# Zilong-Li/BaseVarC

Measured on AMD Instinct MI355X. Metric: sites/sec at N=1e6 samples; achieved HBM GB/s vs roofline, higher is better.
Workload: dtype f64

## Files before the change

basevarc_amd/csrc/bvc_context.hip:

```cpp
#include <cmath>
#include <cstdlib>
#include <cstring>
#include <mutex>
#include <new>

#include "bvc_ctx.h"

hipError_t sync_streams(bvc_ctx *ctx)
{
    hipError_t first = hipSuccess;
    for (hipStream_t s : streams_of(ctx)) {
        const hipError_t e = hipStreamSynchronize(s);
        if (first == hipSuccess) first = e;
    }
    for (bool &p : ctx->em_pending) p = false;
    return first;
}

int drain_on_error(bvc_ctx *ctx, int code)
{
    (void)sync_streams(ctx);
    (void)hipGetLastError();
    return code;
}
// ... 81 lines not shown
        if (c >= r.first && c + n <= r.first + r.second) return true;
    return false;
}

namespace {
struct Knob {
    const char *key, *env;
    int lo, hi, step, dflt;
    int LaunchState::*member;
    bool takes(int v) const { return v >= lo && v <= hi && (v - lo) % step == 0; }
};
const Knob kKnobs[] = {
    {"em_waves_per_cu", "BVC_EM_WAVES_PER_CU", 0, 32, 1, 0, &LaunchState::em_waves_per_cu},
    {"em_wpb", "BVC_EM_WPB", 1, 4, 3, 4, &LaunchState::em_wpb},
    {"hist_split", "BVC_HIST_SPLIT", 0, 64, 1, 0, &LaunchState::hist_split},
    {"group_pipe", "BVC_GROUP_PIPE", 0, 1, 1, 1, &LaunchState::group_pipe},
    {"group_copies_log2", "BVC_GROUP_LOG2C", -1, 5, 1, -1, &LaunchState::group_log2c},
    {"group_big_lds", "BVC_GROUP_BIG_LDS", 0, 1, 1, 1, &LaunchState::group_big_lds},
    {"group_h16", "BVC_GROUP_H16", 0, 1, 1, 0, &LaunchState::group_h16},
    {"em_streams", "BVC_EM_STREAMS", 0, 3, 1, 0, &LaunchState::em_streams},
    {"em_engine", "BVC_EM_ENGINE", 0, 1, 1, 0, &LaunchState::em_engine},
    {"em_tiny_regions", "BVC_EM_TINY_REGIONS", 0, 1, 1, 0, &LaunchState::em_tiny_regions},
    {"em_prune", "BVC_EM_PRUNE", 0, 1, 1, 1, &LaunchState::em_prune},
    {"host_chunk_kib", nullptr, 1, 1 << 21, 1, 1 << 19, &LaunchState::host_chunk_kib},
};
}

extern "C" {

const char *bvc_version(void) { return "libbvc 0.3.0 (gfx950)"; }
// ... 252 lines not shown
```

basevarc_amd/csrc/bvc_internal.h:

```cpp
#pragma once
#include <hip/hip_runtime.h>
#include <stdint.h>

#include <vector>

#include "../../include/bvc.h"

namespace bvc {

struct LaunchState {
    int n_cu = 256;
    int em_waves_per_cu = 0;
    int em_wpb = 4;
    int hist_split = 0;
    int host_chunk_kib = 1 << 19;
    int em_streams = 0;
    int group_pipe = 1;
    int group_log2c = -1;
    int group_big_lds = 1;
    int group_h16 = 0;
    int em_engine = 0;
    int em_tiny_regions = 0;
    int em_prune = 1;
    int dbg_levels = 0;
    mutable uint32_t em_epoch = 0;
    struct RaisedLds { const void *kernel; size_t bytes; };
    mutable std::vector<RaisedLds> lds_raised;
};

// ... 8 lines not shown
        at += round256(count * sizeof(T) + pad);
        return p;
    }
};

hipError_t raise_lds(const LaunchState &st, const void *kernel, size_t bytes);

struct QualLut {
    double a[128];
    double e[128];
    double e_empty;
    double log_e[128];
    double log_a[128];
};

hipError_t launch_hist_dense(LaunchState &st, hipStream_t stream, int64_t n_sites, int64_t n_samples, int64_t row_stride,
                             const int8_t *bases, const int8_t *quals, const uint8_t *group_of_sample,
                             int n_groups, uint32_t *counts, int split, int64_t *group_scratch = nullptr,
                             uint8_t *hist_of_sample = nullptr);
constexpr int kGroupScratchWords = BVC_MAX_GROUPS + 4;
inline size_t group_redo_offset(int64_t n_samples) { return ((size_t)n_samples + 255) & ~(size_t)255; }
inline size_t group_labels_bytes(int64_t n_samples, int64_t n_sites) { return group_redo_offset(n_samples) + (size_t)n_sites + 256; }
int choose_hist_split(const LaunchState &st, int64_t n_sites, int64_t n_samples);

hipError_t launch_hist_packed(LaunchState &st, hipStream_t stream, int64_t n_sites, int64_t n_samples, int64_t row_stride,
                              const uint8_t *packed, uint32_t *counts, int split);
hipError_t launch_hist_packed_groups(LaunchState &st, hipStream_t stream, int64_t n_sites, int64_t n_samples,
                                     int64_t row_stride, const uint8_t *packed, const uint8_t *group_of_sample, int n_groups,
                                     uint32_t *counts, int64_t *group_scratch, uint8_t *hist_of_sample);
hipError_t launch_pack_dense(hipStream_t stream, int64_t n_sites, int64_t n_samples, int64_t stride_in, const int8_t *bases,
                             const int8_t *quals, int64_t stride_out, uint8_t *packed, unsigned long long *bad);

hipError_t launch_stream_read(hipStream_t stream, const void *src, int64_t bytes, uint32_t *sink);

hipError_t launch_hist_csr(LaunchState &st, hipStream_t stream, int64_t n_sites, const int64_t *offsets,
                           const int8_t *bases, const int8_t *quals, uint32_t *counts);

inline bool uses_item_engine(const LaunchState &st, double min_af) { return st.em_engine != 1 && min_af > 0.0; }
hipError_t launch_lrt(const LaunchState &st, hipStream_t stream, int64_t n_sites, const uint32_t *counts,
                      int64_t hist_stride, const int8_t *ref_base, double min_af, const QualLut *lut,
                      const int8_t *comb, const uint8_t *n_comb, bvc_site_result *results, bool shared = false,
// ... 75 lines not shown
```

basevarc_amd/csrc/bvc_lrt.hip:

```cpp
#include "bvc_ctx.h"

namespace {

int em_stream_count(const bvc_ctx *ctx, int by_default) { return ctx->ls.em_streams > 0 ? ctx->ls.em_streams : by_default; }

hipStream_t em_stream(bvc_ctx *ctx, int by_default)
{
    const int n = em_stream_count(ctx, by_default);
    const int k = (int)(ctx->side_flip++ % (unsigned)n);
    return k == 0 ? ctx->side : (k == 1 ? ctx->side_b : ctx->side_c);
}

int ensure_joined(bvc_ctx *ctx, DevBuf &buf, size_t need)
{
    if (need > buf.cap) {
        const int rc = join_side(ctx);
        if (rc != BVC_OK) return rc;
    }
    return ensure(ctx, buf, need);
}

int em_scratch_for(bvc_ctx *ctx, int slot, int64_t n_sites, double min_af, void **out, int n_groups = 0)
{
    *out = nullptr;
    if (!uses_item_engine(ctx->ls, min_af)) return BVC_OK;
    const size_t need = n_groups > 0 ? em_group_scratch_bytes(n_sites, n_groups) : em_items_scratch_bytes(n_sites);
    DevBuf &buf = n_groups > 0 ? ctx->d_emg[slot] : ctx->d_em[slot];
    const int rc = ensure_joined(ctx, buf, need);
    if (rc != BVC_OK) return rc;
    *out = buf.p;
    return BVC_OK;
}

template <class Stage1, class Stage2>
int run_stages(bvc_ctx *ctx, int64_t n_sites, int n_groups, bool zero_counts, double min_af, int em_streams, Stage1 stage1,
               Stage2 stage2)
{
    const size_t cbytes = (size_t)n_sites * BVC_NCLASS * sizeof(uint32_t), gbytes = cbytes * (size_t)(n_groups + 1);
    const int buf = ctx->overlap ? ctx->flip : 0;
    if (ctx->overlap) ctx->flip = (ctx->flip + 1) % bvc_ctx::kRing;
    DevBuf &cnt = ctx->d_cnt[buf], &grp = ctx->d_grp[buf];
    int rc = ensure_joined(ctx, cnt, cbytes);
    if (rc == BVC_OK && n_groups > 0) rc = ensure_joined(ctx, grp, gbytes);
    RingSlot slot;
    if (rc == BVC_OK) rc = em_scratch_for(ctx, buf, n_sites, min_af, &slot.em);
    if (rc == BVC_OK && n_groups > 0) rc = em_scratch_for(ctx, buf, n_sites, min_af, &slot.emg, n_groups);
    if (rc != BVC_OK) return rc;
    slot.counts = reinterpret_cast<uint32_t *>(cnt.p);
    if (n_groups > 0) slot.grp = reinterpret_cast<uint32_t *>(grp.p);
    bvc_ctx::Triple t{nullptr, nullptr, nullptr, nullptr, n_sites};
    const bool timed = ctx->profiling && take_timing_events(ctx, t);
    auto enqueue = [&]() -> int {
        if (ctx->overlap && ctx->em_pending[buf]) {
            BVC_HIP(ctx, hipStreamWaitEvent(ctx->stream, ctx->ev_em_done[buf], 0));
            ctx->em_pending[buf] = false;
        }
        if (zero_counts) BVC_HIP(ctx, hipMemsetAsync(slot.counts, 0, cbytes, ctx->stream));
        if (timed) BVC_HIP(ctx, hipEventRecord(t.a, ctx->stream));
        BVC_HIP(ctx, stage1(n_groups > 0 ? slot.grp : slot.counts));
        if (timed) BVC_HIP(ctx, hipEventRecord(t.b, ctx->stream));
        hipStream_t s2 = ctx->stream;
        if (ctx->overlap) {
            s2 = em_stream(ctx, em_streams);
            BVC_HIP(ctx, hipEventRecord(ctx->ev_hist_done[buf], ctx->stream));
            BVC_HIP(ctx, hipStreamWaitEvent(s2, ctx->ev_hist_done[buf], 0));
        }
        if (timed) BVC_HIP(ctx, hipEventRecord(t.c, s2));
        const int rc2 = stage2(s2, slot);
        if (rc2 != BVC_OK) return rc2;
        if (timed) {
            BVC_HIP(ctx, hipEventRecord(t.d, s2));
            ctx->ev_pending.push_back(t);
            t = bvc_ctx::Triple{nullptr, nullptr, nullptr, nullptr, 0};
            if (ctx->ev_pending.size() > 256) reap_timing(ctx, false);
        }
        if (ctx->overlap) {
            BVC_HIP(ctx, hipEventRecord(ctx->ev_em_done[buf], s2));
            ctx->em_pending[buf] = true;
        }
        return BVC_OK;
    };
    rc = enqueue();
    give_back(ctx, t);
    return rc;
}

template <class Stage1>
int run_two_stages(bvc_ctx *ctx, int64_t n_sites, bool zero_counts, bool long_rows, Stage1 stage1,
                   const int8_t *ref_base, double min_af, const int8_t *comb, const uint8_t *n_comb,
                   bvc_site_result *results, int em_streams_long_rows = 1)
{
    return run_stages(ctx, n_sites, 0, zero_counts, min_af, long_rows ? em_streams_long_rows : 2, stage1,
                      [&](hipStream_t s2, const RingSlot &slot) -> int {
                          const bool shared = ctx->overlap && long_rows;
                          BVC_HIP(ctx, launch_lrt(ctx->ls, s2, n_sites, slot.counts, BVC_NCLASS, ref_base, min_af, ctx->d_lut, comb,
                                                  n_comb, results, shared, 0, slot.em));
                          return BVC_OK;
                      });
}

int run_dense_device(bvc_ctx *ctx, int64_t n_sites, int64_t n_samples, int64_t row_stride,
                     const int8_t *bases, const int8_t *quals, const int8_t *ref_base, double min_af,
                     bvc_site_result *results)
{
    const int split = choose_hist_split(ctx->ls, n_sites, n_samples);
    return run_two_stages(ctx, n_sites, split > 1, n_samples >= 200000,
                          [&](uint32_t *counts) {
                              return launch_hist_dense(ctx->ls, ctx->stream, n_sites, n_samples, row_stride, bases, quals,
                                                       nullptr, 0, counts, split);
                          },
                          ref_base, min_af, nullptr, nullptr, results);
}

int run_packed_device(bvc_ctx *ctx, int64_t n_sites, int64_t n_samples, int64_t row_stride, const uint8_t *packed,
                      const int8_t *ref_base, double min_af, bvc_site_result *results)
{
    const int split = choose_hist_split(ctx->ls, n_sites, n_samples);
    return run_two_stages(ctx, n_sites, split > 1, n_samples >= 200000,
                          [&](uint32_t *counts) {
                              return launch_hist_packed(ctx->ls, ctx->stream, n_sites, n_samples, row_stride, packed, counts, split);
                          },
                          ref_base, min_af, nullptr, nullptr, results, 2);
}

template <class Upload, class Compute>
int run_chunks(bvc_ctx *ctx, int64_t n_sites, int64_t chunk, Upload upload, Compute compute)
{
    int set = 0;
    int rc = upload(set, (int64_t)0, n_sites < chunk ? n_sites : chunk);
    if (rc != BVC_OK) return drain_on_error(ctx, rc);
    BVC_HIP_D(ctx, hipEventRecord(ctx->ev_upload[set], ctx->copy));
    for (int64_t s0 = 0; s0 < n_sites; s0 += chunk, set ^= 1) {
        const int64_t ns = n_sites - s0 < chunk ? n_sites - s0 : chunk;
// ... 61 lines not shown
                int rc = device(ns, d);
                return rc == BVC_OK ? join_side(ctx) : rc;
            }
            BVC_HIP(ctx, hipMemcpyAsync(results + s0, d.res, (size_t)ns * sizeof(bvc_site_result), hipMemcpyDeviceToHost, ctx->stream));
            if (n_groups > 0)
                BVC_HIP(ctx, hipMemcpyAsync(grp_results + s0 * n_groups, d.gres, (size_t)ns * n_groups * sizeof(bvc_group_result),
                                            hipMemcpyDeviceToHost, ctx->stream));
            return BVC_OK;
        });
}

template <class Stage1>
int run_group_stages(bvc_ctx *ctx, int64_t ns, int n_groups, bool long_rows, Stage1 stage1, const int8_t *r, double min_af,
                     bvc_site_result *res, bvc_group_result *gres)
{
    return run_stages(ctx, ns, n_groups, false, min_af, 2, stage1, [&](hipStream_t s2, const RingSlot &slot) -> int {
        BVC_HIP(ctx, launch_sum_groups(s2, ns, n_groups + 1, slot.grp, slot.counts));
        const bool shared = ctx->overlap && long_rows;
        const int per_launch = kGroupSharedWavesPerCu / em_stream_count(ctx, 2) > 2 ? kGroupSharedWavesPerCu / em_stream_count(ctx, 2) : 2;
        BVC_HIP(ctx, launch_lrt(ctx->ls, s2, ns, slot.counts, BVC_NCLASS, r, min_af, ctx->d_lut, nullptr, nullptr, res, shared, per_launch,
                                slot.em));
        BVC_HIP(ctx, launch_lrt_groups(ctx->ls, s2, ns, n_groups, slot.grp, r, min_af, ctx->d_lut, res, gres, shared, per_launch, slot.emg));
        return BVC_OK;
    });
}

int run_csr_groups_device(bvc_ctx *ctx, int64_t n_sites, const int64_t *offsets, const int8_t *bases, const int8_t *quals,
                          const int32_t *sample_of_obs, const int8_t *ref_base, double min_af, const uint8_t *group_of_sample,
                          int64_t n_samples, int32_t n_groups, bvc_site_result *results, bvc_group_result *grp_results)
{
    return run_group_stages(ctx, n_sites, n_groups, false,
// ... 25 lines not shown
    if (rc != BVC_OK) return rc;
    BVC_HIP_D(ctx, hipMemcpyAsync(d_o, offsets, (size_t)(n_sites + 1) * 8, hipMemcpyHostToDevice, ctx->stream));
    BVC_HIP_D(ctx, hipMemcpyAsync(d_r, ref_base, (size_t)n_sites, hipMemcpyHostToDevice, ctx->stream));
    if (n_samples) BVC_HIP_D(ctx, hipMemcpyAsync(d_g, group_of_sample, (size_t)n_samples, hipMemcpyHostToDevice, ctx->stream));
    for (int a = 0; a < n_arrays && total; ++a)
        BVC_HIP_D(ctx, hipMemcpyAsync(arrays[a].dev, arrays[a].host, total * arrays[a].elem, hipMemcpyHostToDevice, ctx->stream));
    rc = device(d_o, d_r, d_g, d_res, d_gres);
    if (rc == BVC_OK) rc = join_side(ctx);
    if (rc != BVC_OK) return drain_on_error(ctx, rc);
    BVC_HIP_D(ctx, hipMemcpyAsync(results, d_res, (size_t)n_sites * sizeof(bvc_site_result), hipMemcpyDeviceToHost, ctx->stream));
    BVC_HIP_D(ctx, hipMemcpyAsync(grp_results, d_gres, (size_t)n_sites * n_groups * sizeof(bvc_group_result), hipMemcpyDeviceToHost, ctx->stream));
    BVC_HIP_D(ctx, hipStreamSynchronize(ctx->stream));
    return BVC_OK;
}

}

int run_csr_device(bvc_ctx *ctx, int64_t n_sites, const int64_t *offsets, const int8_t *bases, const int8_t *quals,
                   const int8_t *ref_base, double min_af, const int8_t *comb, const uint8_t *n_comb,
                   bvc_site_result *results)
{
    return run_two_stages(ctx, n_sites, false, false,
                          [&](uint32_t *counts) { return launch_hist_csr(ctx->ls, ctx->stream, n_sites, offsets, bases, quals, counts); },
                          ref_base, min_af, comb, n_comb, results);
}

int run_csr_labels_device(bvc_ctx *ctx, int64_t n_sites, const int64_t *offsets, const uint8_t *obs, const uint8_t *quals,
                          const uint8_t *group_of_obs, const int8_t *ref_base, double min_af, int32_t n_groups,
                          bvc_site_result *results, bvc_group_result *grp_results)
{
    return run_group_stages(ctx, n_sites, n_groups, false,
                            [&](uint32_t *gp) {
                                return launch_hist_csr_labels(ctx->ls, ctx->stream, n_sites, offsets, obs, quals, group_of_obs, n_groups, gp);
                            },
                            ref_base, min_af, results, grp_results);
}

// ... 49 lines not shown
    BVC_HIP(ctx, launch_pack_dense(ctx->stream, n_sites, n_samples, row_stride, bases, quals, packed_stride, packed, d_bad));
    unsigned long long bad = 0;
    BVC_HIP(ctx, hipMemcpyAsync(&bad, d_bad, sizeof bad, hipMemcpyDeviceToHost, ctx->stream));
    BVC_HIP(ctx, hipStreamSynchronize(ctx->stream));
    *n_unrepresentable = (int64_t)bad;
    return BVC_OK;
}

int bvc_hist_dense_packed(bvc_ctx *ctx, int64_t n_sites, int64_t n_samples, int64_t row_stride, const uint8_t *packed,
                          uint32_t *counts, uint32_t flags)
{
    int rc = check_dense(ctx, n_sites, n_samples, row_stride, n_samples ? (const void *)packed : (const void *)counts, counts, counts, counts);
    if (rc != BVC_OK) return rc;
    if (!(flags & BVC_PTR_DEVICE)) return fail(ctx, BVC_ERR_ARG, "bvc_hist_dense_packed takes device pointers");
    if (n_sites == 0) return BVC_OK;
    const int split = choose_hist_split(ctx->ls, n_sites, n_samples);
    if (split > 1) BVC_HIP(ctx, hipMemsetAsync(counts, 0, (size_t)n_sites * BVC_NCLASS * sizeof(uint32_t), ctx->stream));
    BVC_HIP(ctx, launch_hist_packed(ctx->ls, ctx->stream, n_sites, n_samples, row_stride, packed, counts, split));
    return BVC_OK;
}

int bvc_hist_dense(bvc_ctx *ctx, int64_t n_sites, int64_t n_samples, int64_t row_stride,
                   const int8_t *bases, const int8_t *quals, uint32_t *counts, uint32_t flags)
{
    int rc = check_dense(ctx, n_sites, n_samples, row_stride, n_samples ? (const void *)bases : (const void *)counts,
                         n_samples ? (const void *)quals : (const void *)counts, counts, counts);
    if (rc != BVC_OK) return rc;
    if (n_sites == 0) return BVC_OK;
    const int split = choose_hist_split(ctx->ls, n_sites, n_samples);
    const size_t cbytes = (size_t)n_sites * BVC_NCLASS * sizeof(uint32_t);
    if (flags & BVC_PTR_DEVICE) {
        if (split > 1) BVC_HIP(ctx, hipMemsetAsync(counts, 0, cbytes, ctx->stream));
        BVC_HIP(ctx, launch_hist_dense(ctx->ls, ctx->stream, n_sites, n_samples, row_stride, bases, quals, nullptr, 0, counts, split));
        return BVC_OK;
    }
    const size_t bytes = n_samples ? (size_t)(n_sites - 1) * (size_t)row_stride + (size_t)n_samples : 0;
    int8_t *d_b, *d_q;
    uint32_t *d_c;
    rc = carve(ctx, ctx->d_stage[0], 256, [&](Layout &L) {
        d_b = L.take<int8_t>(bytes);
        d_q = L.take<int8_t>(bytes);
        d_c = L.take<uint32_t>((size_t)n_sites * BVC_NCLASS);
    });
    if (rc != BVC_OK) return rc;
    if (bytes) BVC_HIP(ctx, hipMemcpyAsync(d_b, bases, bytes, hipMemcpyHostToDevice, ctx->stream));
    if (bytes) BVC_HIP(ctx, hipMemcpyAsync(d_q, quals, bytes, hipMemcpyHostToDevice, ctx->stream));
    if (split > 1) BVC_HIP(ctx, hipMemsetAsync(d_c, 0, cbytes, ctx->stream));
    BVC_HIP(ctx, launch_hist_dense(ctx->ls, ctx->stream, n_sites, n_samples, row_stride, d_b, d_q, nullptr, 0, d_c, split));
    BVC_HIP(ctx, hipMemcpyAsync(counts, d_c, cbytes, hipMemcpyDeviceToHost, ctx->stream));
    BVC_HIP(ctx, hipStreamSynchronize(ctx->stream));
    return BVC_OK;
}

static int check_comb_host(bvc_ctx *ctx, int64_t n_sites, const int8_t *base_comb, const uint8_t *n_comb)
{
    for (int64_t s = 0; s < n_sites; ++s) {
        if (n_comb[s] > 4) return fail(ctx, BVC_ERR_ARG, "n_comb > 4");
        for (int c = 0; c < n_comb[s]; ++c)
            if (base_comb[s * 4 + c] < 0 || base_comb[s * 4 + c] > 3) return fail(ctx, BVC_ERR_ARG, "base_comb entry outside 0..3");
    }
    return BVC_OK;
}
// ... 246 lines not shown
    if (n_groups < 1 || n_groups > BVC_MAX_GROUPS) return fail(ctx, BVC_ERR_ARG, "n_groups must be 1..32");
    if (!group_of_sample || !grp_results) return fail(ctx, BVC_ERR_ARG, "null group pointer");
    if (n_sites == 0) return BVC_OK;
    auto run_device = [&](int64_t ns, const int8_t *b, const int8_t *q, const int8_t *r, const uint8_t *g,
                          bvc_site_result *res, bvc_group_result *gres) -> int {
        const size_t lbytes = group_labels_bytes(n_samples, ns);
        int rc2 = ensure_joined(ctx, ctx->d_grp_labels, lbytes);
        if (rc2 != BVC_OK) return rc2;
        uint8_t *labels = reinterpret_cast<uint8_t *>(ctx->d_grp_labels.p);
        return run_group_stages(ctx, ns, n_groups, n_samples >= 200000,
                                [&](uint32_t *gp) {
                                    if (packed)
                                        return launch_hist_packed_groups(ctx->ls, ctx->stream, ns, n_samples, row_stride,
                                                                         reinterpret_cast<const uint8_t *>(b), g, n_groups, gp,
                                                                         ctx->d_grp_scratch, labels);
                                    return launch_hist_dense(ctx->ls, ctx->stream, ns, n_samples, row_stride, b, q, g, n_groups, gp, 1,
                                                             ctx->d_grp_scratch, labels);
                                },
                                r, min_af, res, gres);
    };

    if (flags & BVC_PTR_DEVICE)
        return run_device(n_sites, bases, quals, ref_base, group_of_sample, results, grp_results);

    const int8_t *rows[2] = {bases, quals};
    return run_dense_host(ctx, n_sites, n_samples, row_stride, packed ? 1 : 2, rows, ref_base, group_of_sample, n_groups, results,
                          grp_results, [&](int64_t ns, const DenseSet &d) {
                              return run_device(ns, d.rows[0], d.rows[1], d.ref, d.labels, d.res, d.gres);
                          });
}

// ... 20 lines not shown
```

basevarc_amd/csrc/hist_kernel.hip:

```cpp
#include "bvc_device.h"
#include "bvc_internal.h"

#include <utility>

namespace bvc {
namespace {

#ifndef BVC_HIST_THREADS
#define BVC_HIST_THREADS 512
#endif
#ifndef BVC_HIST_UNROLL
#define BVC_HIST_UNROLL 2
#endif
constexpr int kHistThreads = BVC_HIST_THREADS;
constexpr int kCopies = 32;
constexpr int kLdsWords = BVC_NCLASS * kCopies;
constexpr int kUnroll = BVC_HIST_UNROLL;
constexpr int kGroupDepth = 2;
constexpr int64_t kWaveRowMax = 16384;

typedef uint32_t u32x4 __attribute__((ext_vector_type(4)));

template <int BYTE>
__device__ __forceinline__ uint32_t shl_byte(uint32_t word, uint32_t shift)
// ... 193 lines not shown
        const int64_t c = cb + tid + (int64_t)u * kHistThreads;
        b[u] = u32x4{0xFFFFFFFFu, 0xFFFFFFFFu, 0xFFFFFFFFu, 0xFFFFFFFFu};
        q[u] = u32x4{0u, 0u, 0u, 0u};
        if (c < c1) {
            b[u] = __builtin_nontemporal_load(&bv[c]);
            q[u] = __builtin_nontemporal_load(&qv[c]);
        }
    }
#pragma unroll
    for (int u = 0; u < kUnroll; ++u) {
        const int64_t wave_first = cb + (tid & ~63) + (int64_t)u * kHistThreads;
        if (wave_first < c1) count_chunk(hist, b[u], q[u], lane_off);
    }
}

template <bool ALIGNED>
__global__ __launch_bounds__(kHistThreads) void hist_dense_kernel(
    int64_t n_sites, int64_t n_samples, int64_t row_stride, const int8_t *__restrict__ bases,
    const int8_t *__restrict__ quals, uint32_t *__restrict__ counts, int split)
{
    BVC_POISON_LDS();
    extern __shared__ __attribute__((aligned(16))) uint32_t hist[];
    const int tid = threadIdx.x;
    const uint32_t lane_off = (uint32_t)(tid & (kCopies - 1));
    __builtin_amdgcn_s_setprio(3);

    clear_lds(hist, kLdsWords, tid);
    __syncthreads();

    const int64_t n_work = n_sites * split;
    for (int64_t w = blockIdx.x; w < n_work; w += gridDim.x) {
        const int64_t site = w / split;
        const int part = (int)(w % split);
        const int8_t *brow = bases + site * row_stride;
        const int8_t *qrow = quals + site * row_stride;
        const int64_t n16 = n_samples >> 4;
        constexpr int64_t kBlockChunks = (int64_t)kUnroll * kHistThreads;

        if (ALIGNED) {
            const u32x4 *bv = reinterpret_cast<const u32x4 *>(brow);
            const u32x4 *qv = reinterpret_cast<const u32x4 *>(qrow);
            for (int64_t cb = (int64_t)part * kBlockChunks; cb < n16; cb += (int64_t)split * kBlockChunks) {
                if (cb + kBlockChunks <= n16) {
                    u32x4 b[kUnroll], q[kUnroll];
                    load_block(bv, qv, cb + tid, b, q);
#pragma unroll
                    for (int u = 0; u < kUnroll; ++u) count_chunk(hist, b[u], q[u], lane_off);
                } else {
// ... 4 lines not shown
            for (int64_t cb = (int64_t)part * kBlockChunks; cb < n16; cb += (int64_t)split * kBlockChunks) {
                const int64_t i1 = (cb + kBlockChunks < n16 ? cb + kBlockChunks : n16) * 16;
                count_bytes(hist, brow, qrow, cb * 16, i1, tid, lane_off);
            }
        }
        if (part == split - 1) count_bytes(hist, brow, qrow, n16 << 4, n_samples, tid, lane_off);
        __syncthreads();

        for (int key = tid; key < BVC_NCLASS; key += kHistThreads) {
            const uint32_t s = fold_class<kCopies>(hist, key);
            if (split == 1) counts[site * BVC_NCLASS + key] = s;
            else if (s) atomicAdd(&counts[site * BVC_NCLASS + key], s);
        }
        __syncthreads();
    }
}


__global__ __launch_bounds__(kHistThreads) void hist_dense_groups_bytes_kernel(
    int64_t n_sites, int64_t n_samples, int64_t row_stride, const int8_t *__restrict__ bases,
    const int8_t *__restrict__ quals, const uint8_t *__restrict__ group_of_sample, int n_groups, int log2c,
    uint32_t *__restrict__ grp_counts, const int64_t *__restrict__ bounds)
{
    BVC_POISON_LDS();
    extern __shared__ __attribute__((aligned(16))) uint32_t hist[];
    if (bounds && bounds[0] == 0) return;
    const int tid = threadIdx.x;
    const int n_hist = n_groups + 1;
    const int words = (n_hist * BVC_NCLASS) << log2c;
    const uint32_t lane_off = (uint32_t)tid & ((1u << log2c) - 1u);
// ... 457 lines not shown
{
    for (int64_t i = i0 + tid; i < i1; i += kHistThreads) lds_add_one(((uint32_t)row[i] << 8) + lane_base);
}

__device__ __forceinline__ uint32_t fold_packed_class(uint32_t *hist, int key)
{
    const int q = key & 127;
    if (q >= 64) return 0;
    const uint32_t sum = fold_class<kPackedCopies>(hist, ((key >> 7) << 6) | q);
    return q == 63 ? 0u : sum;
}

template <bool ALIGNED>
__global__ __launch_bounds__(kHistThreads) void hist_packed_kernel(
    int64_t n_sites, int64_t n_samples, int64_t row_stride, const uint8_t *__restrict__ packed,
    uint32_t *__restrict__ counts, int split)
{
    BVC_POISON_LDS();
    extern __shared__ __attribute__((aligned(16))) uint32_t hist[];
    const int tid = threadIdx.x;
    const uint32_t lane_base = lds_address(hist) + ((uint32_t)(tid & (kPackedCopies - 1)) << 2);
    const bool at_zero = (lds_address(hist) & 0xFFFFu) == 0u;
    __builtin_amdgcn_s_setprio(3);
    clear_lds(hist, kPackedLdsWords, tid);
    __syncthreads();

    uint32_t a0 = lane_base, a1 = lane_base, a2 = lane_base, a3 = lane_base;
    const int64_t n_work = n_sites * split;
    for (int64_t w = blockIdx.x; w < n_work; w += gridDim.x) {
        const int64_t site = w / split;
        const int part = (int)(w % split);
        const uint8_t *row = packed + site * row_stride;
        const int64_t n16 = (ALIGNED && at_zero) ? n_samples >> 4 : 0;
        constexpr int64_t kBlockChunks = (int64_t)kPackedUnroll * kHistThreads;
        if (ALIGNED && at_zero) {
            const u32x4 *rv = reinterpret_cast<const u32x4 *>(row);
            for (int64_t cb = (int64_t)part * kBlockChunks; cb < n16; cb += (int64_t)split * kBlockChunks) {
                u32x4 v[kPackedUnroll];
                if (cb + kBlockChunks <= n16) {
                    load_block(rv, cb + tid, v);
                } else {
                    load_partial_block(rv, cb + tid, n16, v);
                }
#pragma unroll
                for (int u = 0; u < kPackedUnroll; ++u) {
                    count_packed_chunk(a0, a1, a2, a3, v[u]);
                }
            }
        }
        if (part == split - 1)
            for (int64_t i = (n16 << 4) + tid; i < n_samples; i += kHistThreads)
                lds_add_one(((uint32_t)row[i] << 8) + lane_base);
        __syncthreads();
        for (int key = tid; key < BVC_NCLASS; key += kHistThreads) {
            const uint32_t sum = fold_packed_class(hist, key);
            if (split == 1) counts[site * BVC_NCLASS + key] = sum;
            else if (sum) atomicAdd(&counts[site * BVC_NCLASS + key], sum);
        }
        __syncthreads();
    }
}

template <bool ALIGNED>
__global__ __launch_bounds__(kHistThreads) void hist_packed_ranges_kernel(
    int64_t n_sites, int64_t row_stride, const uint8_t *__restrict__ packed, int n_hist,
    const int64_t *__restrict__ scratch, uint32_t *__restrict__ grp_counts)
{
    BVC_POISON_LDS();
    extern __shared__ __attribute__((aligned(16))) uint32_t hist[];
    if (scratch[0] != 0) return;
    uint8_t *real_h = reinterpret_cast<uint8_t *>(&hist[kPackedLdsWords]);
    int &n_real_s = *reinterpret_cast<int *>(&hist[kPackedLdsWords + 16]);
    const int tid = threadIdx.x;
    const uint32_t lane_base = lds_address(hist) + ((uint32_t)(tid & (kPackedCopies - 1)) << 2);
    const bool at_zero = (lds_address(hist) & 0xFFFFu) == 0u;
// ... 367 lines not shown
    for (; i + 3 * stride < n16; i += 4 * stride) {
        const u32x4 a = __builtin_nontemporal_load(&src[i]), b = __builtin_nontemporal_load(&src[i + stride]);
        const u32x4 c = __builtin_nontemporal_load(&src[i + 2 * stride]), d = __builtin_nontemporal_load(&src[i + 3 * stride]);
        acc ^= a.x ^ a.y ^ a.z ^ a.w ^ b.x ^ b.y ^ b.z ^ b.w ^ c.x ^ c.y ^ c.z ^ c.w ^ d.x ^ d.y ^ d.z ^ d.w;
    }
    for (; i < n16; i += stride) { const u32x4 a = __builtin_nontemporal_load(&src[i]); acc ^= a.x ^ a.y ^ a.z ^ a.w; }
    if (acc == 0x9E3779B9u) sink[0] = acc;
}

}

#ifdef BVC_CHECK_LDS
BVC_DEFINE_DEBUG_READER(debug_read_hist)
#endif

hipError_t launch_stream_read(hipStream_t stream, const void *src, int64_t bytes, uint32_t *sink)
{
    const int64_t n16 = bytes / 16;
    if (n16 <= 0) return hipSuccess;
    int64_t blocks = (n16 + 4 * 512 - 1) / (4 * 512);
    if (blocks > 16384) blocks = 16384;
    hipLaunchKernelGGL(stream_read_kernel, dim3((unsigned)blocks), dim3(512), 0, stream, reinterpret_cast<const u32x4 *>(src), n16, sink);
    return hipGetLastError();
}

int choose_hist_split(const LaunchState &st, int64_t n_sites, int64_t n_samples)
{
    if (st.hist_split > 0) return st.hist_split;
    const int64_t want = (int64_t)st.n_cu * 4;
    if (n_sites >= want || n_samples < (1 << 16)) return 1;
    int64_t split = (want + n_sites - 1) / n_sites;
    const int64_t max_split = n_samples / (1 << 15);
    if (split > max_split) split = max_split;
    if (split < 1) split = 1;
    if (split > 64) split = 64;
    return (int)split;
}

hipError_t raise_lds(const LaunchState &st, const void *kernel, size_t bytes)
{
    for (LaunchState::RaisedLds &done : st.lds_raised)
        if (done.kernel == kernel) {
            if (done.bytes >= bytes) return hipSuccess;
            const hipError_t e = hipFuncSetAttribute(kernel, hipFuncAttributeMaxDynamicSharedMemorySize, (int)bytes);
            if (e == hipSuccess) done.bytes = bytes;
            return e;
        }
    const hipError_t e = hipFuncSetAttribute(kernel, hipFuncAttributeMaxDynamicSharedMemorySize, (int)bytes);
    if (e == hipSuccess) st.lds_raised.push_back({kernel, bytes});
    return e;
}

constexpr size_t kLdsBytes = (size_t)kLdsWords * sizeof(uint32_t);
static_assert(kPackedLdsWords == kLdsWords, "kLdsBytes serves the packed kernels too");
constexpr size_t kBigLdsBytes = 144 * 1024;
constexpr size_t kGroupLdsMax = (size_t)(BVC_MAX_GROUPS + 1) * BVC_NCLASS * sizeof(uint32_t);

static unsigned grid_cap(int64_t n, int64_t cap = 4096) { return (unsigned)(n < cap ? n : cap); }

template <class... P, class... A>
static hipError_t launch(const LaunchState &st, hipStream_t stream, void (*kernel)(P...), unsigned grid, int block, size_t lds,
                         size_t attr_bytes, A... args)
{
    if (attr_bytes) {
        const hipError_t e = raise_lds(st, reinterpret_cast<const void *>(kernel), attr_bytes);
        if (e != hipSuccess) return e;
    }
    hipLaunchKernelGGL(kernel, dim3(grid), dim3(block), lds, stream, static_cast<P>(args)...);
    return hipGetLastError();
}

using Log2cs = std::make_integer_sequence<int, 6>;
template <bool PIPE, int... L>
// ... 31 lines not shown
                                int n_groups, int64_t *group_scratch, uint8_t *hist_of_sample, int slots, size_t big_tail,
                                Ranges launch_ranges, GroupPlan *plan)
{
    if (!group_scratch || !hist_of_sample) return hipErrorInvalidValue;
    hipError_t e = hipMemsetAsync(group_scratch, 0, (size_t)kGroupScratchWords * sizeof(int64_t), stream);
    if (e != hipSuccess) return e;
    e = launch(st, stream, group_bounds_kernel, grid_cap((n_samples + 255) / 256, 1024), 256, 0, 0, group_of_sample, n_samples,
               n_groups, group_scratch, hist_of_sample);
    if (e != hipSuccess) return e;
    *plan = plan_group_copies(st, n_groups + 1, slots, big_tail);
    return launch_ranges();
}

hipError_t launch_hist_dense(LaunchState &st, hipStream_t stream, int64_t n_sites, int64_t n_samples, int64_t row_stride,
                             const int8_t *bases, const int8_t *quals, const uint8_t *group_of_sample,
                             int n_groups, uint32_t *counts, int split, int64_t *group_scratch, uint8_t *hist_of_sample)
{
    if (n_sites <= 0) return hipSuccess;
    const bool aligned = ((reinterpret_cast<uintptr_t>(bases) | reinterpret_cast<uintptr_t>(quals)) & 15u) == 0 &&
                         (row_stride & 15) == 0;
    if (group_of_sample) {
        const int n_hist = n_groups + 1;
        if (n_samples <= 0)
            return hipMemsetAsync(counts, 0, (size_t)n_sites * n_hist * BVC_NCLASS * sizeof(uint32_t), stream);
        GroupPlan g;
        hipError_t e = group_prelude(st, stream, group_of_sample, n_samples, n_groups, group_scratch, hist_of_sample, BVC_NCLASS, 16, [&] {
            return launch(st, stream, aligned ? hist_dense_ranges_kernel<true> : hist_dense_ranges_kernel<false>,
                          grid_cap(n_sites * n_hist), kHistThreads, kLdsBytes, kLdsBytes, n_sites, n_samples, row_stride, bases, quals,
                          n_hist, group_scratch, counts);
        }, &g);
        if (e != hipSuccess) return e;
// ... 1 lines not shown
            return launch(st, stream, hist_dense_groups_bytes_kernel, grid_cap(n_sites), kHistThreads, g.lds, kGroupLdsMax, n_sites,
                          n_samples, row_stride, bases, quals, group_of_sample, n_groups, g.log2c, counts, group_scratch);
        const uint8_t *only = nullptr;
        if (g.big >= 0 && g.log2c < 3) {
            uint8_t *redo = hist_of_sample + group_redo_offset(n_samples);
            e = launch(st, stream, g.big == 4 ? hist_dense_groups_slots_kernel<4> : (g.big == 3 ? hist_dense_groups_slots_kernel<3> : hist_dense_groups_slots_kernel<2>),
                       grid_cap(n_sites), 1024, g.big_lds, kBigLdsBytes, n_sites, n_samples, row_stride, bases, quals, hist_of_sample,
                       n_groups, counts, group_scratch, redo);
            if (e != hipSuccess) return e;
            only = redo;
        }
        return launch(st, stream, st.group_pipe ? dense_groups_instance<true>(g.log2c, Log2cs{}) : dense_groups_instance<false>(g.log2c, Log2cs{}),
                      grid_cap(n_sites), kHistThreads, g.lds, kGroupLdsMax, n_sites, n_samples, row_stride, bases, quals, hist_of_sample,
                      n_groups, counts, group_scratch, only);
    }
    if (split == 1 && n_samples <= kWaveRowMax && n_sites >= (int64_t)st.n_cu * 2 * kCsrWaves)
        return launch(st, stream, aligned ? hist_wave_kernel<true, true> : hist_wave_kernel<false, true>,
                      grid_cap((n_sites + kCsrWaves - 1) / kCsrWaves, 8192), kHistThreads, 0, 0, n_sites, nullptr, n_samples, row_stride,
                      bases, quals, counts);
    return launch(st, stream, aligned ? hist_dense_kernel<true> : hist_dense_kernel<false>, grid_cap(n_sites * split), kHistThreads,
                  kLdsBytes, kLdsBytes, n_sites, n_samples, row_stride, bases, quals, counts, split);
}

hipError_t launch_hist_packed(LaunchState &st, hipStream_t stream, int64_t n_sites, int64_t n_samples, int64_t row_stride,
                              const uint8_t *packed, uint32_t *counts, int split)
{
    if (n_sites <= 0) return hipSuccess;
    const bool aligned = (reinterpret_cast<uintptr_t>(packed) & 15u) == 0 && (row_stride & 15) == 0;
    return launch(st, stream, aligned ? hist_packed_kernel<true> : hist_packed_kernel<false>, grid_cap(n_sites * split), kHistThreads,
                  kLdsBytes, kLdsBytes, n_sites, n_samples, row_stride, packed, counts, split);
}

hipError_t launch_hist_packed_groups(LaunchState &st, hipStream_t stream, int64_t n_sites, int64_t n_samples,
                                     int64_t row_stride, const uint8_t *packed, const uint8_t *group_of_sample, int n_groups,
                                     uint32_t *counts, int64_t *group_scratch, uint8_t *hist_of_sample)
{
    if (n_sites <= 0) return hipSuccess;
    const int n_hist = n_groups + 1;
    if (n_samples <= 0)
        return hipMemsetAsync(counts, 0, (size_t)n_sites * n_hist * BVC_NCLASS * sizeof(uint32_t), stream);
    const bool aligned = (reinterpret_cast<uintptr_t>(packed) & 15u) == 0 && (row_stride & 15) == 0;
    GroupPlan g;
    hipError_t e = group_prelude(st, stream, group_of_sample, n_samples, n_groups, group_scratch, hist_of_sample, kPackedSlots, 0, [&] {
        return launch(st, stream, aligned ? hist_packed_ranges_kernel<true> : hist_packed_ranges_kernel<false>, grid_cap(n_sites * n_hist),
                      kHistThreads, kLdsBytes + 256, kLdsBytes + 256, n_sites, row_stride, packed, n_hist, group_scratch, counts);
// ... 44 lines not shown
```

Before: 3.340 million.

## Split only tail sites across blocks in histogram kernels to balance last wave

Replaces the uniform per-site split factor with a HistSplit that processes most sites whole and splits only the remainder sites (n_sites mod 2*n_cu) into several parts. This targets the tail-wave imbalance where the last partial wave of blocks leaves CUs idle. Only the split rows are zeroed before the kernel, rather than the whole counts buffer. In exchange, tail sites need atomic accumulation into global counts and some launches get larger grids. A compile-time clock probe is also added.

```diff
diff --git a/basevarc_amd/csrc/bvc_context.hip b/basevarc_amd/csrc/bvc_context.hip
--- a/basevarc_amd/csrc/bvc_context.hip
+++ b/basevarc_amd/csrc/bvc_context.hip
@@ -119,6 +119,7 @@
     {"em_waves_per_cu", "BVC_EM_WAVES_PER_CU", 0, 32, 1, 0, &LaunchState::em_waves_per_cu},
     {"em_wpb", "BVC_EM_WPB", 1, 4, 3, 4, &LaunchState::em_wpb},
     {"hist_split", "BVC_HIST_SPLIT", 0, 64, 1, 0, &LaunchState::hist_split},
+    {"hist_tail_split", "BVC_HIST_TAIL_SPLIT", 0, 64, 1, 0, &LaunchState::hist_tail_split},
     {"group_pipe", "BVC_GROUP_PIPE", 0, 1, 1, 1, &LaunchState::group_pipe},
     {"group_copies_log2", "BVC_GROUP_LOG2C", -1, 5, 1, -1, &LaunchState::group_log2c},
     {"group_big_lds", "BVC_GROUP_BIG_LDS", 0, 1, 1, 1, &LaunchState::group_big_lds},
diff --git a/basevarc_amd/csrc/bvc_internal.h b/basevarc_amd/csrc/bvc_internal.h
--- a/basevarc_amd/csrc/bvc_internal.h
+++ b/basevarc_amd/csrc/bvc_internal.h
@@ -13,6 +13,7 @@
     int em_waves_per_cu = 0;
     int em_wpb = 4;
     int hist_split = 0;
+    int hist_tail_split = 0;
     int host_chunk_kib = 1 << 19;
     int em_streams = 0;
     int group_pipe = 1;
@@ -51,17 +52,18 @@
     double log_a[128];
 };
 
+struct HistSplit { int64_t n_whole; int parts; };
 hipError_t launch_hist_dense(LaunchState &st, hipStream_t stream, int64_t n_sites, int64_t n_samples, int64_t row_stride,
                              const int8_t *bases, const int8_t *quals, const uint8_t *group_of_sample,
-                             int n_groups, uint32_t *counts, int split, int64_t *group_scratch = nullptr,
+                             int n_groups, uint32_t *counts, HistSplit hs, int64_t *group_scratch = nullptr,
                              uint8_t *hist_of_sample = nullptr);
 constexpr int kGroupScratchWords = BVC_MAX_GROUPS + 4;
 inline size_t group_redo_offset(int64_t n_samples) { return ((size_t)n_samples + 255) & ~(size_t)255; }
 inline size_t group_labels_bytes(int64_t n_samples, int64_t n_sites) { return group_redo_offset(n_samples) + (size_t)n_sites + 256; }
-int choose_hist_split(const LaunchState &st, int64_t n_sites, int64_t n_samples);
+HistSplit choose_hist_split(const LaunchState &st, int64_t n_sites, int64_t n_samples);
 
 hipError_t launch_hist_packed(LaunchState &st, hipStream_t stream, int64_t n_sites, int64_t n_samples, int64_t row_stride,
-                              const uint8_t *packed, uint32_t *counts, int split);
+                              const uint8_t *packed, uint32_t *counts, HistSplit hs);
 hipError_t launch_hist_packed_groups(LaunchState &st, hipStream_t stream, int64_t n_sites, int64_t n_samples,
                                      int64_t row_stride, const uint8_t *packed, const uint8_t *group_of_sample, int n_groups,
                                      uint32_t *counts, int64_t *group_scratch, uint8_t *hist_of_sample);
diff --git a/basevarc_amd/csrc/bvc_lrt.hip b/basevarc_amd/csrc/bvc_lrt.hip
--- a/basevarc_amd/csrc/bvc_lrt.hip
+++ b/basevarc_amd/csrc/bvc_lrt.hip
@@ -33,7 +33,7 @@
 }
 
 template <class Stage1, class Stage2>
-int run_stages(bvc_ctx *ctx, int64_t n_sites, int n_groups, bool zero_counts, double min_af, int em_streams, Stage1 stage1,
+int run_stages(bvc_ctx *ctx, int64_t n_sites, int n_groups, int64_t zero_from, double min_af, int em_streams, Stage1 stage1,
                Stage2 stage2)
 {
     const size_t cbytes = (size_t)n_sites * BVC_NCLASS * sizeof(uint32_t), gbytes = cbytes * (size_t)(n_groups + 1);
@@ -55,7 +55,9 @@
             BVC_HIP(ctx, hipStreamWaitEvent(ctx->stream, ctx->ev_em_done[buf], 0));
             ctx->em_pending[buf] = false;
         }
-        if (zero_counts) BVC_HIP(ctx, hipMemsetAsync(slot.counts, 0, cbytes, ctx->stream));
+        if (zero_from < n_sites)
+            BVC_HIP(ctx, hipMemsetAsync(slot.counts + zero_from * BVC_NCLASS, 0, (size_t)(n_sites - zero_from) * BVC_NCLASS * sizeof(uint32_t),
+                                        ctx->stream));
         if (timed) BVC_HIP(ctx, hipEventRecord(t.a, ctx->stream));
         BVC_HIP(ctx, stage1(n_groups > 0 ? slot.grp : slot.counts));
         if (timed) BVC_HIP(ctx, hipEventRecord(t.b, ctx->stream));
@@ -86,11 +88,11 @@
 }
 
 template <class Stage1>
-int run_two_stages(bvc_ctx *ctx, int64_t n_sites, bool zero_counts, bool long_rows, Stage1 stage1,
+int run_two_stages(bvc_ctx *ctx, int64_t n_sites, int64_t zero_from, bool long_rows, Stage1 stage1,
                    const int8_t *ref_base, double min_af, const int8_t *comb, const uint8_t *n_comb,
                    bvc_site_result *results, int em_streams_long_rows = 1)
 {
-    return run_stages(ctx, n_sites, 0, zero_counts, min_af, long_rows ? em_streams_long_rows : 2, stage1,
+    return run_stages(ctx, n_sites, 0, zero_from, min_af, long_rows ? em_streams_long_rows : 2, stage1,
                       [&](hipStream_t s2, const RingSlot &slot) -> int {
                           const bool shared = ctx->overlap && long_rows;
                           BVC_HIP(ctx, launch_lrt(ctx->ls, s2, n_sites, slot.counts, BVC_NCLASS, ref_base, min_af, ctx->d_lut, comb,
@@ -103,8 +105,8 @@
                      const int8_t *bases, const int8_t *quals, const int8_t *ref_base, double min_af,
                      bvc_site_result *results)
 {
-    const int split = choose_hist_split(ctx->ls, n_sites, n_samples);
-    return run_two_stages(ctx, n_sites, split > 1, n_samples >= 200000,
+    const HistSplit split = choose_hist_split(ctx->ls, n_sites, n_samples);
+    return run_two_stages(ctx, n_sites, split.n_whole, n_samples >= 200000,
                           [&](uint32_t *counts) {
                               return launch_hist_dense(ctx->ls, ctx->stream, n_sites, n_samples, row_stride, bases, quals,
                                                        nullptr, 0, counts, split);
@@ -115,8 +117,8 @@
 int run_packed_device(bvc_ctx *ctx, int64_t n_sites, int64_t n_samples, int64_t row_stride, const uint8_t *packed,
                       const int8_t *ref_base, double min_af, bvc_site_result *results)
 {
-    const int split = choose_hist_split(ctx->ls, n_sites, n_samples);
-    return run_two_stages(ctx, n_sites, split > 1, n_samples >= 200000,
+    const HistSplit split = choose_hist_split(ctx->ls, n_sites, n_samples);
+    return run_two_stages(ctx, n_sites, split.n_whole, n_samples >= 200000,
                           [&](uint32_t *counts) {
                               return launch_hist_packed(ctx->ls, ctx->stream, n_sites, n_samples, row_stride, packed, counts, split);
                           },
@@ -208,7 +210,7 @@
 int run_group_stages(bvc_ctx *ctx, int64_t ns, int n_groups, bool long_rows, Stage1 stage1, const int8_t *r, double min_af,
                      bvc_site_result *res, bvc_group_result *gres)
 {
-    return run_stages(ctx, ns, n_groups, false, min_af, 2, stage1, [&](hipStream_t s2, const RingSlot &slot) -> int {
+    return run_stages(ctx, ns, n_groups, ns, min_af, 2, stage1, [&](hipStream_t s2, const RingSlot &slot) -> int {
         BVC_HIP(ctx, launch_sum_groups(s2, ns, n_groups + 1, slot.grp, slot.counts));
         const bool shared = ctx->overlap && long_rows;
         const int per_launch = kGroupSharedWavesPerCu / em_stream_count(ctx, 2) > 2 ? kGroupSharedWavesPerCu / em_stream_count(ctx, 2) : 2;
@@ -264,13 +266,19 @@
     return BVC_OK;
 }
 
+hipError_t zero_split_rows(hipStream_t stream, uint32_t *counts, int64_t n_sites, const HistSplit &hs)
+{
+    if (hs.n_whole >= n_sites) return hipSuccess;
+    return hipMemsetAsync(counts + hs.n_whole * BVC_NCLASS, 0, (size_t)(n_sites - hs.n_whole) * BVC_NCLASS * sizeof(uint32_t), stream);
+}
+
 }
 
 int run_csr_device(bvc_ctx *ctx, int64_t n_sites, const int64_t *offsets, const int8_t *bases, const int8_t *quals,
                    const int8_t *ref_base, double min_af, const int8_t *comb, const uint8_t *n_comb,
                    bvc_site_result *results)
 {
-    return run_two_stages(ctx, n_sites, false, false,
+    return run_two_stages(ctx, n_sites, n_sites, false,
                           [&](uint32_t *counts) { return launch_hist_csr(ctx->ls, ctx->stream, n_sites, offsets, bases, quals, counts); },
                           ref_base, min_af, comb, n_comb, results);
 }
@@ -350,8 +358,8 @@
     if (rc != BVC_OK) return rc;
     if (!(flags & BVC_PTR_DEVICE)) return fail(ctx, BVC_ERR_ARG, "bvc_hist_dense_packed takes device pointers");
     if (n_sites == 0) return BVC_OK;
-    const int split = choose_hist_split(ctx->ls, n_sites, n_samples);
-    if (split > 1) BVC_HIP(ctx, hipMemsetAsync(counts, 0, (size_t)n_sites * BVC_NCLASS * sizeof(uint32_t), ctx->stream));
+    const HistSplit split = choose_hist_split(ctx->ls, n_sites, n_samples);
+    BVC_HIP(ctx, zero_split_rows(ctx->stream, counts, n_sites, split));
     BVC_HIP(ctx, launch_hist_packed(ctx->ls, ctx->stream, n_sites, n_samples, row_stride, packed, counts, split));
     return BVC_OK;
 }
@@ -363,10 +371,10 @@
                          n_samples ? (const void *)quals : (const void *)counts, counts, counts);
     if (rc != BVC_OK) return rc;
     if (n_sites == 0) return BVC_OK;
-    const int split = choose_hist_split(ctx->ls, n_sites, n_samples);
+    const HistSplit split = choose_hist_split(ctx->ls, n_sites, n_samples);
     const size_t cbytes = (size_t)n_sites * BVC_NCLASS * sizeof(uint32_t);
     if (flags & BVC_PTR_DEVICE) {
-        if (split > 1) BVC_HIP(ctx, hipMemsetAsync(counts, 0, cbytes, ctx->stream));
+        BVC_HIP(ctx, zero_split_rows(ctx->stream, counts, n_sites, split));
         BVC_HIP(ctx, launch_hist_dense(ctx->ls, ctx->stream, n_sites, n_samples, row_stride, bases, quals, nullptr, 0, counts, split));
         return BVC_OK;
     }
@@ -381,7 +389,7 @@
     if (rc != BVC_OK) return rc;
     if (bytes) BVC_HIP(ctx, hipMemcpyAsync(d_b, bases, bytes, hipMemcpyHostToDevice, ctx->stream));
     if (bytes) BVC_HIP(ctx, hipMemcpyAsync(d_q, quals, bytes, hipMemcpyHostToDevice, ctx->stream));
-    if (split > 1) BVC_HIP(ctx, hipMemsetAsync(d_c, 0, cbytes, ctx->stream));
+    BVC_HIP(ctx, zero_split_rows(ctx->stream, d_c, n_sites, split));
     BVC_HIP(ctx, launch_hist_dense(ctx->ls, ctx->stream, n_sites, n_samples, row_stride, d_b, d_q, nullptr, 0, d_c, split));
     BVC_HIP(ctx, hipMemcpyAsync(counts, d_c, cbytes, hipMemcpyDeviceToHost, ctx->stream));
     BVC_HIP(ctx, hipStreamSynchronize(ctx->stream));
@@ -658,7 +666,7 @@
                                         return launch_hist_packed_groups(ctx->ls, ctx->stream, ns, n_samples, row_stride,
                                                                          reinterpret_cast<const uint8_t *>(b), g, n_groups, gp,
                                                                          ctx->d_grp_scratch, labels);
-                                    return launch_hist_dense(ctx->ls, ctx->stream, ns, n_samples, row_stride, b, q, g, n_groups, gp, 1,
+                                    return launch_hist_dense(ctx->ls, ctx->stream, ns, n_samples, row_stride, b, q, g, n_groups, gp, HistSplit{ns, 1},
                                                              ctx->d_grp_scratch, labels);
                                 },
                                 r, min_af, res, gres);
diff --git a/basevarc_amd/csrc/hist_kernel.hip b/basevarc_amd/csrc/hist_kernel.hip
--- a/basevarc_amd/csrc/hist_kernel.hip
+++ b/basevarc_amd/csrc/hist_kernel.hip
@@ -231,12 +231,38 @@
     }
 }
 
+#ifdef BVC_HIST_CLOCKS
+constexpr unsigned kClockSlots = 40960;
+__device__ unsigned long long g_hist_clocks[2 * kClockSlots];
+#define BVC_HIST_CLOCK(which)                                                                                      \
+    do {                                                                                                           \
+        if (threadIdx.x == 0 && blockIdx.x < kClockSlots) g_hist_clocks[2 * blockIdx.x + (which)] = wall_clock64(); \
+    } while (0)
+#else
+#define BVC_HIST_CLOCK(which) do { } while (0)
+#endif
+
+struct HistItem { int64_t site; int part, split; };
+
+__device__ __forceinline__ int64_t hist_item_count(int64_t n_sites, int64_t n_whole, int tail_split)
+{
+    return n_whole + (n_sites - n_whole) * tail_split;
+}
+
+__device__ __forceinline__ HistItem hist_item(int64_t w, int64_t n_whole, int tail_split)
+{
+    if (w < n_whole) return {w, 0, 1};
+    const int64_t t = w - n_whole;
+    return {n_whole + t / tail_split, (int)(t % tail_split), tail_split};
+}
+
 template <bool ALIGNED>
 __global__ __launch_bounds__(kHistThreads) void hist_dense_kernel(
     int64_t n_sites, int64_t n_samples, int64_t row_stride, const int8_t *__restrict__ bases,
-    const int8_t *__restrict__ quals, uint32_t *__restrict__ counts, int split)
+    const int8_t *__restrict__ quals, uint32_t *__restrict__ counts, int64_t n_whole, int tail_split)
 {
     BVC_POISON_LDS();
+    BVC_HIST_CLOCK(0);
     extern __shared__ __attribute__((aligned(16))) uint32_t hist[];
     const int tid = threadIdx.x;
     const uint32_t lane_off = (uint32_t)(tid & (kCopies - 1));
@@ -245,10 +271,11 @@
     clear_lds(hist, kLdsWords, tid);
     __syncthreads();
 
-    const int64_t n_work = n_sites * split;
+    const int64_t n_work = hist_item_count(n_sites, n_whole, tail_split);
     for (int64_t w = blockIdx.x; w < n_work; w += gridDim.x) {
-        const int64_t site = w / split;
-        const int part = (int)(w % split);
+        const HistItem item = hist_item(w, n_whole, tail_split);
+        const int64_t site = item.site;
+        const int part = item.part, split = item.split;
         const int8_t *brow = bases + site * row_stride;
         const int8_t *qrow = quals + site * row_stride;
         const int64_t n16 = n_samples >> 4;
@@ -283,6 +310,7 @@
         }
         __syncthreads();
     }
+    BVC_HIST_CLOCK(1);
 }
 
 
@@ -770,9 +798,10 @@
 template <bool ALIGNED>
 __global__ __launch_bounds__(kHistThreads) void hist_packed_kernel(
     int64_t n_sites, int64_t n_samples, int64_t row_stride, const uint8_t *__restrict__ packed,
-    uint32_t *__restrict__ counts, int split)
+    uint32_t *__restrict__ counts, int64_t n_whole, int tail_split)
 {
     BVC_POISON_LDS();
+    BVC_HIST_CLOCK(0);
     extern __shared__ __attribute__((aligned(16))) uint32_t hist[];
     const int tid = threadIdx.x;
     const uint32_t lane_base = lds_address(hist) + ((uint32_t)(tid & (kPackedCopies - 1)) << 2);
@@ -782,10 +811,11 @@
     __syncthreads();
 
     uint32_t a0 = lane_base, a1 = lane_base, a2 = lane_base, a3 = lane_base;
-    const int64_t n_work = n_sites * split;
+    const int64_t n_work = hist_item_count(n_sites, n_whole, tail_split);
     for (int64_t w = blockIdx.x; w < n_work; w += gridDim.x) {
-        const int64_t site = w / split;
-        const int part = (int)(w % split);
+        const HistItem item = hist_item(w, n_whole, tail_split);
+        const int64_t site = item.site;
+        const int part = item.part, split = item.split;
         const uint8_t *row = packed + site * row_stride;
         const int64_t n16 = (ALIGNED && at_zero) ? n_samples >> 4 : 0;
         constexpr int64_t kBlockChunks = (int64_t)kPackedUnroll * kHistThreads;
@@ -815,6 +845,7 @@
         }
         __syncthreads();
     }
+    BVC_HIST_CLOCK(1);
 }
 
 template <bool ALIGNED>
@@ -1212,6 +1243,24 @@
 BVC_DEFINE_DEBUG_READER(debug_read_hist)
 #endif
 
+#ifdef BVC_HIST_CLOCKS
+}
+extern "C" int bvc_debug_hist_clocks(unsigned long long *out, int max_pairs, int reset)
+{
+    if (!out || max_pairs < 1) return (int)hipErrorInvalidValue;
+    if ((unsigned)max_pairs > bvc::kClockSlots) max_pairs = (int)bvc::kClockSlots;
+    hipError_t e = hipDeviceSynchronize();
+    if (e == hipSuccess) e = hipMemcpyFromSymbol(out, HIP_SYMBOL(bvc::g_hist_clocks), (size_t)max_pairs * 2 * sizeof(unsigned long long));
+    if (e == hipSuccess && reset) {
+        void *p = nullptr;
+        e = hipGetSymbolAddress(&p, HIP_SYMBOL(bvc::g_hist_clocks));
+        if (e == hipSuccess) e = hipMemset(p, 0, sizeof(unsigned long long) * 2 * bvc::kClockSlots);
+    }
+    return (int)e;
+}
+namespace bvc {
+#endif
+
 hipError_t launch_stream_read(hipStream_t stream, const void *src, int64_t bytes, uint32_t *sink)
 {
     const int64_t n16 = bytes / 16;
@@ -1222,17 +1271,30 @@
     return hipGetLastError();
 }
 
-int choose_hist_split(const LaunchState &st, int64_t n_sites, int64_t n_samples)
-{
-    if (st.hist_split > 0) return st.hist_split;
-    const int64_t want = (int64_t)st.n_cu * 4;
-    if (n_sites >= want || n_samples < (1 << 16)) return 1;
-    int64_t split = (want + n_sites - 1) / n_sites;
-    const int64_t max_split = n_samples / (1 << 15);
-    if (split > max_split) split = max_split;
-    if (split < 1) split = 1;
-    if (split > 64) split = 64;
-    return (int)split;
+constexpr int64_t kGridCap = 4096;
+constexpr int64_t kTailFill = 2;
+constexpr int kMaxParts = 64;
+
+HistSplit choose_hist_split(const LaunchState &st, int64_t n_sites, int64_t n_samples)
+{
+    const HistSplit none{n_sites, 1};
+    if (st.hist_split > 0) return st.hist_split > 1 ? HistSplit{0, st.hist_split} : none;
+    const int64_t slots = (int64_t)st.n_cu * 2, tail = n_sites % slots;
+    const bool tail_ok = st.hist_tail_split != 1 && tail > 0 && n_sites <= kGridCap;
+    if (tail_ok && st.hist_tail_split > 1) return HistSplit{n_sites - tail, st.hist_tail_split};
+    int64_t max_parts = n_samples / (1 << 15);
+    if (max_parts > kMaxParts) max_parts = kMaxParts;
+    if (max_parts < 2) return none;
+    if (n_sites < 2 * slots) {
+        int64_t parts = (2 * slots + n_sites - 1) / n_sites;
+        if (parts > max_parts) parts = max_parts;
+        return HistSplit{0, (int)parts};
+    }
+    if (!tail_ok) return none;
+    int64_t parts = 2;
+    while (tail * parts < kTailFill * slots && parts < max_parts) parts *= 2;
+    if (parts > max_parts) parts = max_parts;
+    return HistSplit{n_sites - tail, (int)parts};
 }
 
 hipError_t raise_lds(const LaunchState &st, const void *kernel, size_t bytes)
@@ -1254,7 +1316,13 @@
 constexpr size_t kBigLdsBytes = 144 * 1024;
 constexpr size_t kGroupLdsMax = (size_t)(BVC_MAX_GROUPS + 1) * BVC_NCLASS * sizeof(uint32_t);
 
-static unsigned grid_cap(int64_t n, int64_t cap = 4096) { return (unsigned)(n < cap ? n : cap); }
+static unsigned grid_cap(int64_t n, int64_t cap = kGridCap) { return (unsigned)(n < cap ? n : cap); }
+
+static unsigned grid_for(const HistSplit &hs, int64_t n_sites)
+{
+    const int64_t items = hs.n_whole + (n_sites - hs.n_whole) * hs.parts;
+    return hs.n_whole > 0 && hs.n_whole < n_sites ? (unsigned)items : grid_cap(items);
+}
 
 template <class... P, class... A>
 static hipError_t launch(const LaunchState &st, hipStream_t stream, void (*kernel)(P...), unsigned grid, int block, size_t lds,
@@ -1316,7 +1384,7 @@
 
 hipError_t launch_hist_dense(LaunchState &st, hipStream_t stream, int64_t n_sites, int64_t n_samples, int64_t row_stride,
                              const int8_t *bases, const int8_t *quals, const uint8_t *group_of_sample,
-                             int n_groups, uint32_t *counts, int split, int64_t *group_scratch, uint8_t *hist_of_sample)
+                             int n_groups, uint32_t *counts, HistSplit hs, int64_t *group_scratch, uint8_t *hist_of_sample)
 {
     if (n_sites <= 0) return hipSuccess;
     const bool aligned = ((reinterpret_cast<uintptr_t>(bases) | reinterpret_cast<uintptr_t>(quals)) & 15u) == 0 &&
@@ -1348,21 +1416,21 @@
                       grid_cap(n_sites), kHistThreads, g.lds, kGroupLdsMax, n_sites, n_samples, row_stride, bases, quals, hist_of_sample,
                       n_groups, counts, group_scratch, only);
     }
-    if (split == 1 && n_samples <= kWaveRowMax && n_sites >= (int64_t)st.n_cu * 2 * kCsrWaves)
+    if (hs.n_whole == n_sites && n_samples <= kWaveRowMax && n_sites >= (int64_t)st.n_cu * 2 * kCsrWaves)
         return launch(st, stream, aligned ? hist_wave_kernel<true, true> : hist_wave_kernel<false, true>,
                       grid_cap((n_sites + kCsrWaves - 1) / kCsrWaves, 8192), kHistThreads, 0, 0, n_sites, nullptr, n_samples, row_stride,
                       bases, quals, counts);
-    return launch(st, stream, aligned ? hist_dense_kernel<true> : hist_dense_kernel<false>, grid_cap(n_sites * split), kHistThreads,
-                  kLdsBytes, kLdsBytes, n_sites, n_samples, row_stride, bases, quals, counts, split);
+    return launch(st, stream, aligned ? hist_dense_kernel<true> : hist_dense_kernel<false>, grid_for(hs, n_sites), kHistThreads,
+                  kLdsBytes, kLdsBytes, n_sites, n_samples, row_stride, bases, quals, counts, hs.n_whole, hs.parts);
 }
 
 hipError_t launch_hist_packed(LaunchState &st, hipStream_t stream, int64_t n_sites, int64_t n_samples, int64_t row_stride,
-                              const uint8_t *packed, uint32_t *counts, int split)
+                              const uint8_t *packed, uint32_t *counts, HistSplit hs)
 {
     if (n_sites <= 0) return hipSuccess;
     const bool aligned = (reinterpret_cast<uintptr_t>(packed) & 15u) == 0 && (row_stride & 15) == 0;
-    return launch(st, stream, aligned ? hist_packed_kernel<true> : hist_packed_kernel<false>, grid_cap(n_sites * split), kHistThreads,
-                  kLdsBytes, kLdsBytes, n_sites, n_samples, row_stride, packed, counts, split);
+    return launch(st, stream, aligned ? hist_packed_kernel<true> : hist_packed_kernel<false>, grid_for(hs, n_sites), kHistThreads,
+                  kLdsBytes, kLdsBytes, n_sites, n_samples, row_stride, packed, counts, hs.n_whole, hs.parts);
 }
 
 hipError_t launch_hist_packed_groups(LaunchState &st, hipStream_t stream, int64_t n_sites, int64_t n_samples,
```

Result: no change. 3.354 million, median of 5 (+0.4%).
